# PlasmaControl/spectrogram-enhancement

Measured on AMD Instinct MI355X. Metric: spectrograms/s (STFT+VAE-denoise fwd) at 1/2/4/8 GPUs; PSNR vs CPU ref, higher is better.
Workload: dtype fp16; 1 GPU; BASELINE config 5 per GPU: end-to-end STFT -> SVD -> autoencoder-denoise inference stream, 16,512-sample fp16 shots -> specgr 128x128 (256 hann / hop 128) -> denoiseSignal default -> 3-layer conv AE (16/32/64, 5x5) fp16 forward -> fp16 reconstructions (32,768 B per shot); shots_per_launch=2048, samples=16512, stft_dtype=fp32, svd_dtype=fp32 (fp64 small algebra), ae_dtype=fp16, parallelism=shot-sharded x1, streams_per_gpu=2

## Files before the change

### spectrogram-enhancement_amd/csrc/decoder_tail.hip

```cpp
#include <hip/hip_runtime.h>

#include <algorithm>
#include <cstdlib>
#include <cstdint>
#include <string>
#include <type_traits>
#include <vector>

#include "lds_dma.hpp"
#include "specenh.h"
#include "runtime.hpp"
#include "wave.hpp"

namespace specenh {

namespace {

typedef _Float16 f16x8 __attribute__((ext_vector_type(8)));
typedef __bf16 bf16x8 __attribute__((ext_vector_type(8)));
typedef _Float16 f16x2 __attribute__((ext_vector_type(2)));
typedef __bf16 bf16x2 __attribute__((ext_vector_type(2)));
typedef float f32x4 __attribute__((ext_vector_type(4)));

constexpr int TO = 32;
// ... 500 lines not shown
  }
  if (i < ns) step(IC<0>{}, i, pa);
  if (i + 1 < ns) step(IC<1>{}, i + 1, pb);
  if (i + 2 < ns) step(IC<2>{}, i + 2, pa);
}

#ifndef SPECENH_D3_PEMIT
#define SPECENH_D3_PEMIT 0
#endif
namespace d3 {
constexpr int CI1 = 64, CO1 = 32;
constexpr int W1 = 32;
constexpr int X1ST = CI1;
constexpr int X1ROW = (W1 + 2) * X1ST;
constexpr int NX1 = 8;
constexpr int X2ST = 32;
constexpr int X2ROW = (2 * W1 + 2) * X2ST;
constexpr int NX2 = 8;
constexpr int LDS_X1 = NX1 * X1ROW * 2;
constexpr int LDS_X2 = NX2 * X2ROW * 2;
constexpr int LDS_M = rows::NMR * rows::MROW * 2;
constexpr int LDS_S = 4 * rows::SCR * rows::SCW * 4;
constexpr int LDS_BYTES = LDS_X1 + LDS_X2 + LDS_M + LDS_S;
constexpr int NBND = 6 * 2 * 4;
constexpr int BSTR = NBND + 64;
constexpr int LDS_ES = SPECENH_D3_PEMIT ? 2 * 2 * 4 * 64 * 4 : 0;
constexpr int LDS_BYTES_NM = LDS_X1 + LDS_X2 + 4 * BSTR * 4 + LDS_ES;
}

__device__ __forceinline__ int x1_off(int ps, int g) { return ps * d3::X1ST + 8 * (g ^ (ps & 7)); }

__device__ __forceinline__ int x2_off(int ps, int g) { return ps * d3::X2ST + 8 * (g ^ ((ps >> 1) & 3)); }


#ifndef SPECENH_D3_CPRIO
#define SPECENH_D3_CPRIO 1
#endif
#ifndef SPECENH_D3_BRANCHFREE
#define SPECENH_D3_BRANCHFREE 1
#endif

struct D3Args {
  const void* x;
  const void* w1;
  const float* b1;
  const void* wt;
  const float* bt;
  const void* wo;
  const float* bo;
  void* out;
  int N, H;
  int out_f16;
};

#ifdef SPECENH_D3_STATS
__device__ unsigned long long d3_stats[1024 * 8 * 4];
struct D3Clock {
  long long last = 0, busy = 0, wait = 0, n = 0;
  __device__ __forceinline__ void barrier() {
    asm volatile("s_waitcnt lgkmcnt(0)" ::: "memory");
    const long long t0 = __builtin_amdgcn_s_memtime();
    asm volatile("s_waitcnt lgkmcnt(0)" ::: "memory");
    __builtin_amdgcn_s_barrier();
    asm volatile("" ::: "memory");
    const long long t1 = __builtin_amdgcn_s_memtime();
    asm volatile("s_waitcnt lgkmcnt(0)" ::: "memory");
    if (last) busy += t0 - last;
    wait += t1 - t0;
    ++n;
    last = t1;
  }
  __device__ void flush(int wv) {
    if ((threadIdx.x & 63) == 0 && blockIdx.x < 1024) {
      unsigned long long* p = d3_stats + (blockIdx.x * 8 + wv) * 4;
      p[0] = busy; p[1] = wait; p[2] = n; p[3] = 0;
    }
  }
};
#define D3_BARRIER() clk.barrier()
#else
#define D3_BARRIER() lds_barrier()
#endif

template <typename T, bool MAP, int LEAD, bool OUT16 = false>
__global__ __launch_bounds__(512, 2) void decoder3_kernel(D3Args a) {
  static_assert(LEAD >= 0 && LEAD <= 4, "8-row input ring");
  using namespace d3;
  extern __shared__ __attribute__((aligned(16))) unsigned char lds_raw[];
  constexpr int LB = MAP ? LDS_BYTES : LDS_BYTES_NM;
  T* const x1r = reinterpret_cast<T*>(lds_raw);
  T* const x2r = reinterpret_cast<T*>(lds_raw + LDS_X1);
  T* const mr = reinterpret_cast<T*>(lds_raw + LDS_X1 + LDS_X2);
  float* const sc = reinterpret_cast<float*>(lds_raw + LDS_X1 + LDS_X2 + LDS_M);
  float* const bnd = reinterpret_cast<float*>(lds_raw + LDS_X1 + LDS_X2);
  float* const es = bnd + 4 * BSTR;

  const int tid = threadIdx.x, lane = tid & 63;
  const int wv = __builtin_amdgcn_readfirstlane(tid >> 6);
  const int m = lane & 15, kg = lane >> 4;
  const int H1 = a.H, H2 = 2 * H1, H3 = 4 * H1;
#ifdef SPECENH_D3_STATS
  D3Clock clk;
#endif
  const int SPI = H1 + 1, TPI = 2 * SPI;
  const int G = gridDim.x;
  const int nimg = ((int)a.N - (int)blockIdx.x + G - 1) / G;
  const int S = nimg * SPI + 2;
  {
    uint4* z = reinterpret_cast<uint4*>(lds_raw);
    for (int e = tid; e < LB / 16; e += 512) z[e] = uint4{0u, 0u, 0u, 0u};
  }
  __syncthreads();

  if (wv < 4) {
    const int wx = wv & 1, nb = wv >> 1;
    uint4 w1[50];
    {
      const T* __restrict__ Wg = reinterpret_cast<const T*>(a.w1);
      int u = 0;
#pragma unroll
      for (int ph = 0; ph < 4; ++ph)
#pragma unroll
        for (int dy = -1; dy <= 1; ++dy)
#pragma unroll
          for (int dx = -1; dx <= 1; ++dx) {
            const int ky = ky_of(ph >> 1, dy), kx = ky_of(ph & 1, dx);
            if (ky < 0 || ky >= KT || kx < 0 || kx >= KT) continue;
#pragma unroll
            for (int kh = 0; kh < 2; ++kh)
              w1[u++] = *reinterpret_cast<const uint4*>(
                  Wg + (((16 * nb + m) * KT + ky) * KT + kx) * CI1 + 32 * kh + 8 * kg);
          }
    }
    const f32x4 bias = f32x4{a.b1[16 * nb + 4 * kg], a.b1[16 * nb + 4 * kg + 1],
                             a.b1[16 * nb + 4 * kg + 2], a.b1[16 * nb + 4 * kg + 3]};
    resident_loads_landed();
    const T* __restrict__ X = reinterpret_cast<const T*>(a.x);
    const int dps = 1 + 8 * wv + (lane >> 3);
    const int dsrc = (dps - 1) * CI1 + 8 * ((lane & 7) ^ (dps & 7));
    unsigned char* const ddst = lds_raw + (1 + 8 * wv) * X1ST * 2;
    auto stage_at = [&](int p, int il, int row) -> bool {
      unsigned char* dst = ddst + (p & (NX1 - 1)) * X1ROW * 2;
      if (il < nimg && row >= 0 && row < H1) {
        const long long n = (long long)blockIdx.x + (long long)il * G;
        lds_dma16_s(X + ((n * H1 + row) * W1) * CI1, 2u * dsrc, dst);
        return true;
      }
      *reinterpret_cast<uint4*>(dst + 16 * lane) = uint4{0u, 0u, 0u, 0u};
      return false;
    };
    auto stage = [&](int p) -> bool {
      const int il = p / SPI;
      return stage_at(p, il, p - il * SPI - 1);
    };
    int xo[3];
#pragma unroll
    for (int dx = -1; dx <= 1; ++dx) xo[dx + 1] = x1_off(16 * wx + m + dx + 1, kg);
    const int x2w16 = x2_off(2 * (16 * wx + m) + 1 + (kg & 1), 2 * nb + (kg >> 1));
    auto store_pair = [&](T* row, uint2 p0, uint2 p1) {
      const auto sx = __builtin_amdgcn_permlane16_swap(p0.x, p1.x, false, false);
      const auto sy = __builtin_amdgcn_permlane16_swap(p0.y, p1.y, false, false);
      *reinterpret_cast<uint4*>(row + x2w16) = uint4{sx[0], sy[0], sx[1], sy[1]};
    };
#pragma unroll
    for (int p = 0; p < 3 + LEAD; ++p) stage(p);
    asm volatile("s_waitcnt vmcnt(0)" ::: "memory");
    D3_BARRIER();
    int vmn = 0;
// ... 73 lines not shown
      pstep(IC<6>{}, g + 6);
      pstep(IC<7>{}, g + 7);
    }
    if (g < S) pstep(IC<0>{}, g);
    if (g + 1 < S) pstep(IC<1>{}, g + 1);
    if (g + 2 < S) pstep(IC<2>{}, g + 2);
    if (g + 3 < S) pstep(IC<3>{}, g + 3);
    if (g + 4 < S) pstep(IC<4>{}, g + 4);
    if (g + 5 < S) pstep(IC<5>{}, g + 5);
    if (g + 6 < S) pstep(IC<6>{}, g + 6);
#ifdef SPECENH_D3_STATS
    clk.flush(wv);
#endif
  } else if constexpr (!MAP) {
    const int w = wv - 4;
    uint4 wt[25];
    {
      const T* __restrict__ Wt = reinterpret_cast<const T*>(a.wt);
      int u = 0;
#pragma unroll
      for (int ph = 0; ph < 4; ++ph)
#pragma unroll
        for (int dy = -1; dy <= 1; ++dy)
#pragma unroll
          for (int dx = -1; dx <= 1; ++dx) {
            const int ky = ky_of(ph >> 1, dy), kx = ky_of(ph & 1, dx);
            if (ky < 0 || ky >= KT || kx < 0 || kx >= KT) continue;
            wt[u++] = *reinterpret_cast<const uint4*>(Wt + ((m * KT + ky) * KT + kx) * CI + 8 * kg);
          }
    }
    const f32x4 bias = f32x4{a.bt[4 * kg], a.bt[4 * kg + 1], a.bt[4 * kg + 2], a.bt[4 * kg + 3]};
    uint4 wd[3][2];
    {
      const T* __restrict__ Wo = reinterpret_cast<const T*>(a.wo);
      const int i = lane & 15, kA = lane >> 4;
      const int gO = i >> 2, j = i & 3, r = gO >> 1, o = gO & 1;
      const int ox = o + (j == 1 ? 2 : (j == 2 ? -2 : 0));
#pragma unroll
      for (int d = 0; d < 3; ++d)
#pragma unroll
        for (int py = 0; py < 2; ++py) {
          const int ky = py + 2 - 2 * (d - 1) - r;
          uint32_t e[4];
#pragma unroll
          for (int h = 0; h < 4; ++h) {
            uint32_t v2 = 0;
#pragma unroll
            for (int s2 = 0; s2 < 2; ++s2) {
              const int el = 2 * h + s2, px = el >> 2, c = el & 3, kx = px + 2 - ox;
              unsigned short bits = 0;
              if (j < 3 && ky >= 0 && ky < KO && kx >= 0 && kx < KO)
                bits = __builtin_bit_cast(unsigned short, Wo[(ky * KO + kx) * CO + 4 * kA + c]);
              v2 |= (uint32_t)bits << (16 * s2);
            }
            e[h] = v2;
          }
          wd[d][py] = uint4{e[0], e[1], e[2], e[3]};
        }
    }
    const float bo = a.bo[0];
    resident_loads_landed();
    int xo[3];
#pragma unroll
    for (int dx = -1; dx <= 1; ++dx) xo[dx + 1] = x2_off(16 * w + m + dx + 1, kg);
    const int orow = kg >> 1, ocol = 32 * w + 2 * m + (kg & 1);
    const int bwi = (m == 0 || m == 15) ? ((w + 1) * 2 + (m == 0 ? 1 : 0)) * 4 + kg : NBND + lane;
    const int bri = m == 0 ? (w * 2 + 0) * 4 + kg : (m == 15 ? ((w + 2) * 2 + 1) * 4 + kg : 0);
#if SPECENH_D3_CPRIO
    __builtin_amdgcn_s_setprio(1);
#endif
    D3_BARRIER();

    f32x4 P0 = f32x4{0.f, 0.f, 0.f, 0.f}, P1 = P0, P2 = P0;
    int il = -1, tl = TPI - 4;
    auto frags = [&](auto ic, uint4 (&bq)[9]) {
      constexpr int T8 = decltype(ic)::value;
#pragma unroll
      for (int dy = -1; dy <= 1; ++dy)
#pragma unroll
        for (int dx = -1; dx <= 1; ++dx)
          bq[3 * (dy + 1) + dx + 1] =
              *reinterpret_cast<const uint4*>(x2r + ((T8 + dy + 8) & 7) * X2ROW + xo[dx + 1]);
    };
    auto tstep = [&](auto ic, const uint4 (&bq)[9], float* bb, f32x4& E, int& eil,
                     int& etl) -> bool {
      constexpr int T8 = decltype(ic)::value;
      (void)T8;
      eil = il;
      etl = tl;
      if (++tl == TPI) { tl = 0; ++il; }
      const bool img = eil >= 0 && eil < nimg;
#if !SPECENH_D3_BRANCHFREE
      if (!img) return false;
#endif
      f32x4 acc[4] = {bias, bias, bias, bias};
      int u0[4] = {0, 4, 10, 16};
#pragma unroll
      for (int dy = -1; dy <= 1; ++dy)
#pragma unroll
        for (int dx = -1; dx <= 1; ++dx) {
          const uint4 b = bq[3 * (dy + 1) + dx + 1];
#pragma unroll
          for (int ph = 0; ph < 4; ++ph) {
            const int ky = ky_of(ph >> 1, dy), kx = ky_of(ph & 1, dx);
            if (ky < 0 || ky >= KT || kx < 0 || kx >= KT) continue;
            acc[ph] = mfma<T>(wt[u0[ph]++], b, acc[ph]);
          }
        }
      const uint32_t keep = img && etl < H2 ? 0xffffffffu : 0u;
      uint4 bv[2];
#pragma unroll
      for (int py = 0; py < 2; ++py) {
        const uint2 lo = relu_pack<T>(acc[2 * py]), hi = relu_pack<T>(acc[2 * py + 1]);
        bv[py] = uint4{lo.x & keep, lo.y & keep, hi.x & keep, hi.y & keep};
      }
#pragma unroll
      for (int py = 0; py < 2; ++py) {
        P0 = mfma<T>(wd[0][py], bv[py], P0);
        P1 = mfma<T>(wd[1][py], bv[py], P1);
        P2 = mfma<T>(wd[2][py], bv[py], P2);
      }
      E = P0;
      P0 = P1;
      P1 = P2;
      P2 = f32x4{0.f, 0.f, 0.f, 0.f};
#if SPECENH_D3_BRANCHFREE
      bb[bwi] = m == 0 ? E[2] : E[1];
      return img && etl >= 1 && etl <= H2;
#else
      if (etl < 1 || etl > H2) return false;
      if (m == 0 || m == 15) bb[bwi] = m == 0 ? E[2] : E[1];
      return true;
#endif
    };
    auto tskip = [&](float* bb, f32x4& E, int& eil, int& etl) -> bool {
      eil = il;
      etl = tl;
      if (++tl == TPI) { tl = 0; ++il; }
      E = P0;
      P0 = P1;
      P1 = P2;
      P2 = f32x4{0.f, 0.f, 0.f, 0.f};
      bb[bwi] = m == 0 ? E[2] : E[1];
      return eil >= 0 && eil < nimg && etl >= 1 && etl <= H2;
    };
    auto emit = [&](const f32x4& E, float edge, int eil, int etl) {
      float s = bo + E[0];
      s += dpp_shift<0x111>(E[1]);
      s += dpp_shift<0x101>(E[2]);
      s += edge;
      const long long n = (long long)blockIdx.x + (long long)eil * G;
      const long long o = (n * H3 + 2 * (etl - 1) + orow) * rows::MW + ocol;
      const float y = __builtin_amdgcn_rcpf(1.f + __expf(-s));
      if constexpr (OUT16)
        reinterpret_cast<_Float16*>(a.out)[o] = (_Float16)y;
      else
        reinterpret_cast<float*>(a.out)[o] = y;
    };
    auto cstep = [&](auto ic) {
      constexpr int I = decltype(ic)::value;
      float* const b0 = bnd + ((I & 1) * 2) * BSTR;
      float* const b1 = b0 + BSTR;
      f32x4 E0, E1;
      int il0, tl0, il1, tl1;
      bool e0, e1;
      if (il >= 0 && il < nimg && tl < H2) {
        uint4 bq[9];
        frags(IC<(2 * I + 4) & 7>{}, bq);
        __builtin_amdgcn_sched_barrier(0);
        e0 = tstep(IC<(2 * I + 4) & 7>{}, bq, b0, E0, il0, tl0);
        frags(IC<(2 * I + 5) & 7>{}, bq);
        __builtin_amdgcn_sched_barrier(0);
        e1 = tstep(IC<(2 * I + 5) & 7>{}, bq, b1, E1, il1, tl1);
      } else {
        e0 = tskip(b0, E0, il0, tl0);
        e1 = tskip(b1, E1, il1, tl1);
      }
#if SPECENH_D3_PEMIT
      (void)e0;
      (void)e1;
      float* const ep = es + ((I & 1) * 2 * 4 + w) * 64 + lane;
      ep[0] = ((bo + E0[0]) + dpp_shift<0x111>(E0[1])) + dpp_shift<0x101>(E0[2]);
      ep[4 * 64] = ((bo + E1[0]) + dpp_shift<0x111>(E1[1])) + dpp_shift<0x101>(E1[2]);
      D3_BARRIER();
#else
      D3_BARRIER();
      if (e0) emit(E0, b0[bri], il0, tl0);
      if (e1) emit(E1, b1[bri], il1, tl1);
#endif
    };
    int g = 0;
    for (; g + 4 <= S; g += 4) {
      cstep(IC<0>{});
      cstep(IC<1>{});
      cstep(IC<2>{});
      cstep(IC<3>{});
    }
    if (g < S) cstep(IC<0>{});
    if (g + 1 < S) cstep(IC<1>{});
    if (g + 2 < S) cstep(IC<2>{});
#ifdef SPECENH_D3_STATS
    clk.flush(wv);
#endif
  } else {
    const int w = wv - 4;
    TailWave<T> tw;
    tw.load(a.wt, a.bt, a.wo, a.bo, w, lane);
    int xo[3];
#pragma unroll
    for (int dx = -1; dx <= 1; ++dx) xo[dx + 1] = x2_off(16 * w + m + dx + 1, kg);
    D3_BARRIER();
    auto tstep = [&](auto ic, const int t, float* scb) {
      constexpr int T8 = decltype(ic)::value;
      constexpr int T4 = T8 & 3;
      if (t < 0) return;
      const int il = t / TPI, tl = t - il * TPI;
      if (il >= nimg) return;
      if (tl >= 2)
        tw.conv_out_d([&](int j) { return mr + ((2 * T4 - 6 + j + 8) & 7) * rows::MROW; }, scb,
                      m);
      T* const m0 = mr + ((2 * T4) & 7) * rows::MROW;
      T* const m1 = mr + ((2 * T4 + 1) & 7) * rows::MROW;
      if (tl < H2)
        tw.convt(x2r, [](int dy) { return ((T8 + dy + 8) & 7) * X2ROW; },
                 [&](int dx) { return xo[dx + 1]; }, m0, m1);
      else
        tw.zero_rows(m0, m1);
    };
    auto sums = [&](const float* scb, int t) {
      if (t < 0) return;
      const int il = t / TPI, tl = t - il * TPI;
      if (il >= nimg || tl < 2) return;
      const long long n = (long long)blockIdx.x + (long long)il * G;
      tw.conv_out_sums(scb, reinterpret_cast<float*>(a.out) + n * H3 * rows::MW, 2 * tl - 4,
                       lane);
    };
    auto cstep = [&](auto ic, const int g) {
      constexpr int I = decltype(ic)::value;
      float* const sc0 = sc + ((I & 1) * 2) * (rows::SCR * rows::SCW);
      float* const sc1 = sc0 + rows::SCR * rows::SCW;
      tstep(IC<(2 * I + 5) & 7>{}, 2 * g - 3, sc0);
      tstep(IC<(2 * I + 6) & 7>{}, 2 * g - 2, sc1);
      D3_BARRIER();
      sums(sc0, 2 * g - 3);
      sums(sc1, 2 * g - 2);
    };
    int g = 0;
    for (; g + 4 <= S; g += 4) {
      cstep(IC<0>{}, g);
      cstep(IC<1>{}, g + 1);
      cstep(IC<2>{}, g + 2);
      cstep(IC<3>{}, g + 3);
    }
    if (g < S) cstep(IC<0>{}, g);
    if (g + 1 < S) cstep(IC<1>{}, g + 1);
    if (g + 2 < S) cstep(IC<2>{}, g + 2);
#ifdef SPECENH_D3_STATS
    clk.flush(wv);
#endif
  }
}

}
}

using namespace specenh;

namespace {
template <bool TRAIN>
int launch_tail_rows(int dtype, RowsArgs& r, hipStream_t st) {
  const int N = r.N, H = r.H;
  int nb = 1;
  while (nb < 8 && (long long)N * nb < 2ll * device_cus() && 2 * H / (2 * nb) >= 8) nb *= 2;
  r.R = ((2 * H + nb - 1) / nb + 1) & ~1;
  r.nb = (2 * H + r.R - 1) / r.R;
  const long long grid = (long long)N * r.nb;
  if (grid >= (1ll << 31)) return set_error(SPECENH_EINVAL, "too many workgroups");
  if (dtype == SPECENH_DTYPE_F16)
    SPECENH_LAUNCH((tail_rows_kernel<_Float16, TRAIN>), dim3((unsigned)grid), dim3(256), rows::LDS_BYTES, st, r);
  else
    SPECENH_LAUNCH((tail_rows_kernel<__bf16, TRAIN>), dim3((unsigned)grid), dim3(256), rows::LDS_BYTES, st, r);
  const hipError_t e = hipGetLastError();
  if (e != hipSuccess) return set_error(SPECENH_EHIP, std::string("tail_rows: ") + hipGetErrorString(e));
  return SPECENH_OK;
}
}

extern "C" int specenh_convt_conv_out_train(int dtype, const void* x, int N, int H, int W, int C,
                                            const void* wt_gemm, const float* bt, int CO_, int kt,
                                            const void* wo_gemm, const float* bo, int ko,
                                            void* map, float* logits, void* out, void* stream) {
  if (N < 0 || H <= 0 || W <= 0) return set_error(SPECENH_EINVAL, "bad input shape");
  if (dtype != SPECENH_DTYPE_F16 && dtype != SPECENH_DTYPE_BF16)
    return set_error(SPECENH_EUNSUPPORTED, "fused decoder tail: fp16 / bf16 only");
  if (C != CI || CO_ != CO || kt != KT || ko != KO || W != rows::QW)
    return set_error(SPECENH_EUNSUPPORTED,
                     "fused decoder tail (training): Conv2DTranspose(16, 5) on 64-wide "
                     "32-channel inputs + Conv2D(1, 5)");
  if (N == 0) return SPECENH_OK;
  if (!x || !wt_gemm || !bt || !wo_gemm || !bo || !map || !logits || !out)
    return set_error(SPECENH_EINVAL, "null pointer");
  if ((long long)N * H * W * C >= (1ll << 31) || (long long)N * 4 * H * W * CO >= (1ll << 31))
    return set_error(SPECENH_EINVAL, "tensor too large (2^31 elements)");
  RowsArgs r{};
  r.x = x; r.wt = wt_gemm; r.bt = bt; r.wo = wo_gemm; r.bo = bo;
  r.map = map; r.logits = logits; r.out_t = out;
  r.N = N; r.H = H;
  return launch_tail_rows<true>(dtype, r, (hipStream_t)stream);
}

namespace specenh {
bool tail_rows_general_supported(int C, int CO, int kt, int ko, int W);
int tail_rows_general(int dtype, const void* x, int N, int H, int W, int C, const void* wt,
                      const float* bt, int CO, int kt, const void* wo, const float* bo, int ko,
                      float* out, hipStream_t st, bool* launched);
}

extern "C" int specenh_convt_conv_out(int dtype, const void* x, int N, int H, int W, int C,
                                      const void* wt_gemm, const float* bt, int CO_, int kt,
                                      const void* wo_gemm, const float* bo, int ko, float* out,
                                      void* stream) {
  if (N < 0 || H <= 0 || W <= 0) return set_error(SPECENH_EINVAL, "bad input shape");
  if (dtype != SPECENH_DTYPE_F16 && dtype != SPECENH_DTYPE_BF16)
    return set_error(SPECENH_EUNSUPPORTED, "fused decoder tail: fp16 / bf16 only");
  hipStream_t st = (hipStream_t)stream;
  if (tail_rows_general_supported(C, CO_, kt, ko, W)) {
    if (N == 0) return SPECENH_OK;
    bool launched = false;
    const int rc = tail_rows_general(dtype, x, N, H, W, C, wt_gemm, bt, CO_, kt, wo_gemm, bo, ko,
                                     out, st, &launched);
    if (rc != SPECENH_OK || launched) return rc;
  }
  if (C != CI || CO_ != CO || kt != KT || ko != KO)
    return set_error(SPECENH_EUNSUPPORTED,
                     "fused decoder tail: Conv2DTranspose(16, 5) on 32 channels + Conv2D(1, 5), "
                     "or Conv2DTranspose(32, k) + Conv2D(1, k), k = 3 / 5 / 7, on 64-wide inputs");
  if (N == 0) return SPECENH_OK;
  if (W == rows::QW && variant(V_TAIL_TILES) == 0) {
    if (!x || !wt_gemm || !bt || !wo_gemm || !bo || !out) return set_error(SPECENH_EINVAL, "null pointer");
    if ((long long)N * H * W * C >= (1ll << 31) || (long long)N * 4 * H * W >= (1ll << 31))
      return set_error(SPECENH_EINVAL, "tensor too large (2^31 elements)");
    RowsArgs r{};
    r.x = x; r.wt = wt_gemm; r.bt = bt; r.wo = wo_gemm; r.bo = bo; r.out = out;
    r.N = N; r.H = H;
    return launch_tail_rows<false>(dtype, r, st);
  }
  if (!x || !wt_gemm || !bt || !wo_gemm || !bo || !out) return set_error(SPECENH_EINVAL, "null pointer");
  if ((long long)N * H * W * C >= (1ll << 31) || (long long)N * 4 * H * W >= (1ll << 31))
    return set_error(SPECENH_EINVAL, "tensor too large (2^31 elements)");
  TailArgs a{};
  a.x = x;
  a.wt = wt_gemm;
  a.bt = bt;
  a.wo = wo_gemm;
  a.bo = bo;
  a.out = out;
  a.N = N;
  a.H = H;
  a.W = W;
  a.tiles_y = (2 * H + TO - 1) / TO;
  a.tiles_x = (2 * W + TO - 1) / TO;
  const long long tiles = (long long)N * a.tiles_y * a.tiles_x;
  if (tiles >= (1ll << 31)) return set_error(SPECENH_EINVAL, "too many tiles");
  const unsigned grid = (unsigned)std::min<long long>(tiles, resident_grid());
  if (dtype == SPECENH_DTYPE_F16)
    SPECENH_LAUNCH(convt_conv_out_kernel<_Float16>, dim3(grid), dim3(512), 0, st, a);
  else
    SPECENH_LAUNCH(convt_conv_out_kernel<__bf16>, dim3(grid), dim3(512), 0, st, a);
  const hipError_t e = hipGetLastError();
  if (e != hipSuccess) return set_error(SPECENH_EHIP, std::string("convt_conv_out: ") +
                                                          hipGetErrorString(e));
  return SPECENH_OK;
}

#ifdef SPECENH_D3_STATS
extern "C" int specenh_d3_stats(void* host, int bytes) {
  return hipMemcpyFromSymbol(host, HIP_SYMBOL(d3_stats), bytes) == hipSuccess ? 0 : -1;
}
#endif

extern "C" int specenh_decoder3_ex(int dtype, const void* x, int N, int H, int W, int C,
                                   const void* w1_gemm, const float* b1, int CO1,
                                   const void* wt_gemm, const float* bt, int CO2,
                                   const void* wo_gemm, const float* bo, int k, void* out,
                                   int out_dtype, void* stream) {
  if (out_dtype != SPECENH_DTYPE_F32 && out_dtype != SPECENH_DTYPE_F16)
    return set_error(SPECENH_EUNSUPPORTED, "fused decoder: fp32 or fp16 output");
  if (N < 0 || H <= 0 || W <= 0) return set_error(SPECENH_EINVAL, "bad input shape");
  if (dtype != SPECENH_DTYPE_F16 && dtype != SPECENH_DTYPE_BF16)
    return set_error(SPECENH_EUNSUPPORTED, "fused decoder: fp16 / bf16 only");
  if (W != d3::W1 || C != d3::CI1 || CO1 != d3::CO1 || CO2 != CO || k != KT)
    return set_error(SPECENH_EUNSUPPORTED,
                     "fused decoder: Conv2DTranspose(32, 5) on 32-wide 64-channel inputs + "
                     "Conv2DTranspose(16, 5) + Conv2D(1, 5)");
  if (N == 0) return SPECENH_OK;
  if (!x || !w1_gemm || !b1 || !wt_gemm || !bt || !wo_gemm || !bo || !out)
    return set_error(SPECENH_EINVAL, "null pointer");
  if ((long long)N * H * W * C >= (1ll << 31) || (long long)N * 16 * H * W >= (1ll << 31))
    return set_error(SPECENH_EINVAL, "tensor too large (2^31 elements)");
  D3Args a{};
  a.x = x; a.w1 = w1_gemm; a.b1 = b1; a.wt = wt_gemm; a.bt = bt; a.wo = wo_gemm; a.bo = bo;
  a.out = out; a.N = N; a.H = H;
  a.out_f16 = out_dtype == SPECENH_DTYPE_F16;
  hipStream_t st = (hipStream_t)stream;
  static LdsOptIn lds_map, lds_nm;
  (void)allow_lds(lds_map,
                  {reinterpret_cast<const void*>(&decoder3_kernel<_Float16, true, 0>),
                   reinterpret_cast<const void*>(&decoder3_kernel<__bf16, true, 0>)},
                  d3::LDS_BYTES);
  (void)allow_lds(lds_nm,
                  {reinterpret_cast<const void*>(&decoder3_kernel<_Float16, false, 3>),
                   reinterpret_cast<const void*>(&decoder3_kernel<__bf16, false, 3>),
                   reinterpret_cast<const void*>(&decoder3_kernel<_Float16, false, 0>),
                   reinterpret_cast<const void*>(&decoder3_kernel<__bf16, false, 0>),
                   reinterpret_cast<const void*>(&decoder3_kernel<_Float16, false, 3, true>),
                   reinterpret_cast<const void*>(&decoder3_kernel<__bf16, false, 3, true>),
                   reinterpret_cast<const void*>(&decoder3_kernel<_Float16, false, 0, true>),
                   reinterpret_cast<const void*>(&decoder3_kernel<__bf16, false, 0, true>)},
                  d3::LDS_BYTES_NM);
  const unsigned grid = (unsigned)std::min<long long>(N, device_cus());
  const bool map = variant(V_D3_MAP) != 0, short_lead = variant(V_ROWS_SHORT_LEAD) != 0;
  if (map && a.out_f16)
    return set_error(SPECENH_EUNSUPPORTED, "fused decoder: the map consumer stores fp32 only");
  const dim3 gd(grid), bd(512);
  auto launch_nm = [&](auto t, auto o16) {
    using TT = decltype(t);
    constexpr bool O16 = decltype(o16)::value;
    if (short_lead)
      SPECENH_LAUNCH((decoder3_kernel<TT, false, 0, O16>), gd, bd, d3::LDS_BYTES_NM, st, a);
    else
      SPECENH_LAUNCH((decoder3_kernel<TT, false, 3, O16>), gd, bd, d3::LDS_BYTES_NM, st, a);
  };
  using F16OUT = std::integral_constant<bool, true>;
  using F32OUT = std::integral_constant<bool, false>;
  if (dtype == SPECENH_DTYPE_F16) {
    if (map)
      SPECENH_LAUNCH((decoder3_kernel<_Float16, true, 0>), gd, bd, d3::LDS_BYTES, st, a);
    else if (a.out_f16)
      launch_nm(_Float16{}, F16OUT{});
    else
      launch_nm(_Float16{}, F32OUT{});
  } else {
    if (map)
      SPECENH_LAUNCH((decoder3_kernel<__bf16, true, 0>), gd, bd, d3::LDS_BYTES, st, a);
    else if (a.out_f16)
      launch_nm(__bf16{}, F16OUT{});
    else
      launch_nm(__bf16{}, F32OUT{});
  }
  const hipError_t e = hipGetLastError();
  if (e != hipSuccess) return set_error(SPECENH_EHIP, std::string("decoder3: ") + hipGetErrorString(e));
  return SPECENH_OK;
}

extern "C" int specenh_decoder3(int dtype, const void* x, int N, int H, int W, int C,
                                const void* w1_gemm, const float* b1, int CO1, const void* wt_gemm,
                                const float* bt, int CO2, const void* wo_gemm, const float* bo,
                                int k, float* out, void* stream) {
  return specenh_decoder3_ex(dtype, x, N, H, W, C, w1_gemm, b1, CO1, wt_gemm, bt, CO2, wo_gemm, bo,
                             k, out, SPECENH_DTYPE_F32, stream);
}
```

### spectrogram-enhancement_amd/csrc/runtime.hip

```cpp
#include "runtime.hpp"

#include <algorithm>
#include <atomic>
#include <cstdlib>
#include <cstring>
#include <mutex>
#include <string>

#include "specenh.h"

namespace specenh {
namespace {

struct VariantName {
  const char* name;
  int dflt;
};
constexpr VariantName kVariants[V_COUNT] = {
    {"CONVT_PAIR", 0},      {"PATCH_NO_WL", 0},      {"PATCH_NO_K5", 0},
    {"PATCH_WSPLIT", -1},   {"CONV_NO_S2", 0},       {"CONV_NO_PATCH", 0},
    {"CONV_NO_C1MFMA", 0},  {"CONV_NO_NARROW", 0},   {"WGRAD_GENERIC", 0},
    {"WGRAD_NO_CO1", 0},    {"WGRAD_PERPHASE", 0},   {"SVD_GRAM_TILES", 0},
    {"TAIL_TILES", 0},      {"DECODER_UNFUSED", 0},  {"SVD_NO_TOP1", 0},
    {"CONV_NO_ROWS", 0},    {"CONVT_NO_ROWS", 0},    {"CONV1_NO_ROWS", 0},
    {"ENCODER_UNFUSED", 0},  {"STFT_NO_HOLD", 0},    {"D3_MAP", 0},
    {"ENC2_WPE2", 0},        {"CONVT_SHARED_RING", 0}, {"SVD_RECON_VALU", 0},
    {"ROWS_SHORT_LEAD", 0},  {"SVD_GRAM_F32", 0},
    {"SVD_RECON_BLOCKS", 0}, {"CONVT_PG", 0}, {"SVD_GZ_ROWS", 0}, {"EIG_SPLIT", 0}, {"CO1_VALU", 0},
    {"C1_MASK_MFMA", 1}, {"S2_MIN_NT", 2}, {"PATCH_MIN_WG", 512}, {"WGRAD_WG", 1024}, {"WGRAD_C1_TILES", 4},
    {"EIG_GRID", 32}, {"ROWS_BANDS", -1}, {"CONVT_STORE8", 0},
};

std::atomic<int> g_variant[V_COUNT];
std::once_flag g_variant_once;

void init_variants() {
  for (int i = 0; i < V_COUNT; ++i) {
    int v = kVariants[i].dflt;
    std::string env = std::string("SPECENH_") + kVariants[i].name;
    if (const char* s = std::getenv(env.c_str()); s && *s) v = std::atoi(s);
    g_variant[i].store(v, std::memory_order_relaxed);
  }
}

int variant_index(const char* name) {
  if (!name) return -1;
  if (std::strncmp(name, "SPECENH_", 8) == 0) name += 8;
  for (int i = 0; i < V_COUNT; ++i)
    if (std::strcmp(name, kVariants[i].name) == 0) return i;
  return -1;
}

constexpr int kMaxDevices = 64;
std::atomic<int> g_cus[kMaxDevices];

constexpr int kRing = 256;
thread_local const void* g_ring[kRing];
thread_local long long g_launches = 0;

thread_local std::string g_last_error;

}

int set_error(int code, const std::string& msg) {
  g_last_error = msg;
  return code;
}

int variant(Variant v) {
  std::call_once(g_variant_once, init_variants);
  return g_variant[v].load(std::memory_order_relaxed);
}

int device_cus() {
  int dev = 0;
  if (hipGetDevice(&dev) != hipSuccess || dev < 0 || dev >= kMaxDevices) return 256;
  int c = g_cus[dev].load(std::memory_order_relaxed);
  if (c > 0) return c;
  if (hipDeviceGetAttribute(&c, hipDeviceAttributeMultiprocessorCount, dev) != hipSuccess || c <= 0)
    c = 256;
  g_cus[dev].store(c, std::memory_order_relaxed);
  return c;
}

hipError_t allow_lds(LdsOptIn& site, std::initializer_list<const void*> kernels, int bytes) {
  static_assert(sizeof(site.done) / sizeof(site.done[0]) == kMaxDevices, "one flag per device");
  int dev = 0;
  hipError_t e = hipGetDevice(&dev);
  if (e != hipSuccess) return e;
  const bool known = dev >= 0 && dev < kMaxDevices;
  if (known && site.done[dev].load(std::memory_order_acquire)) return hipSuccess;
  for (const void* k : kernels) {
    hipFuncAttributes fa{};
    e = hipFuncGetAttributes(&fa, k);
    if (e != hipSuccess) return e;
    e = hipFuncSetAttribute(k, hipFuncAttributeMaxDynamicSharedMemorySize,
                            std::min(bytes, 160 * 1024 - (int)fa.sharedSizeBytes));
    if (e != hipSuccess) return e;
  }
  if (known) site.done[dev].store(true, std::memory_order_release);
  return hipSuccess;
}

void note_launch(const void* kernel) { g_ring[g_launches++ % kRing] = kernel; }

}

extern "C" {

const char* specenh_last_error(void) { return specenh::g_last_error.c_str(); }

int specenh_set_variant(const char* name, int value) {
  const int i = specenh::variant_index(name);
// ... 65 lines not shown
```

### spectrogram-enhancement_amd/csrc/runtime.hpp

```cpp
#pragma once

#include <hip/hip_runtime.h>

#include <atomic>
#include <initializer_list>
#include <string>

namespace specenh {

int set_error(int code, const std::string& msg);

inline int ilog2i(int n) {
  int l = 0;
  while ((1 << l) < n) ++l;
  return l;
}

enum Variant : int {
  V_CONVT_PAIR = 0,
  V_PATCH_NO_WL,
  V_PATCH_NO_K5,
  V_PATCH_WSPLIT,
  V_CONV_NO_S2,
  V_CONV_NO_PATCH,
  V_CONV_NO_C1MFMA,
  V_CONV_NO_NARROW,
  V_WGRAD_GENERIC,
  V_WGRAD_NO_CO1,
  V_WGRAD_PERPHASE,
  V_SVD_GRAM_TILES,
  V_TAIL_TILES,
  V_DECODER_UNFUSED,
  V_SVD_NO_TOP1,
  V_CONV_NO_ROWS,
  V_CONVT_NO_ROWS,
  V_CONV1_NO_ROWS,
  V_ENCODER_UNFUSED,
  V_STFT_NO_HOLD,
  V_D3_MAP,
  V_ENC2_WPE2,
  V_CONVT_SHARED_RING,
  V_SVD_RECON_VALU,
  V_ROWS_SHORT_LEAD,
  V_SVD_GRAM_F32,
  V_SVD_RECON_BLOCKS,
  V_CONVT_PG,
  V_SVD_GZ_ROWS,
  V_EIG_SPLIT,
  V_CO1_VALU,
  V_C1_MASK_MFMA,
  V_S2_MIN_NT,
  V_PATCH_MIN_WG,
  V_WGRAD_WG,
  V_WGRAD_C1_TILES,
  V_EIG_GRID,
  V_ROWS_BANDS,
  V_CONVT_STORE8,
  V_COUNT
};

int variant(Variant v);

int device_cus();

struct LdsOptIn {
  std::atomic<bool> done[64];
};
hipError_t allow_lds(LdsOptIn& site, std::initializer_list<const void*> kernels, int bytes);

void note_launch(const void* kernel);

}

#define SPECENH_LAUNCH(K, ...)                                        \
  do {                                                                \
    ::specenh::note_launch(reinterpret_cast<const void*>(&K));        \
    hipLaunchKernelGGL(K, __VA_ARGS__);                               \
  } while (0)
```

### spectrogram-enhancement_amd/csrc/svd_denoise.hip

```cpp
#include <hip/hip_runtime.h>

#include <algorithm>
#include <cmath>
#include <cstdlib>
#include <string>
#include <vector>

#include "fft_common.hpp"
#include "specenh.h"
#include "runtime.hpp"
#include "wave.hpp"

namespace specenh {

typedef float f32x16 __attribute__((ext_vector_type(16)));

struct XView {
  const float* base;
  long long batch_stride;
  long long sk, si;
};

__global__ __launch_bounds__(256) void gram_kernel(XView x, int K, int r, float* G,
                                                   int ntiles_side) {
// ... 2669 lines not shown
                          long long osi, long long nb, hipStream_t st) {
  static LdsOptIn lds_site;
  const hipError_t e = allow_lds(
      lds_site,
      {(const void*)recon_stream_kernel<KP, TO, true>, (const void*)recon_stream_kernel<KP, TO, false>,
       (const void*)recon_mfma_kernel<KP, TO>, (const void*)recon_kernel<KP, TO>},
      kMaxLds);
  if (e != hipSuccess) return e;
  if (variant(V_SVD_RECON_VALU) == 0) {
    constexpr int NT = (KP + 15) / 16, KPP = 16 * NT, KS = 2 * NT < 4 ? 2 : 1;
    const int RP = (r + 15) & ~15;
    const size_t lm = ((size_t)RP * (KPP + 1) + (size_t)RB * (RP + 2) +
                       (size_t)KS * RB * (KPP + 1)) * 4;
    const bool rowmaj16 = xb.si == 1 && r % 4 == 0 && xb.sk % 4 == 0 &&
                          xb.batch_stride % 4 == 0 && (reinterpret_cast<uintptr_t>(xb.base) & 15) == 0;
    const bool trans = xb.sk == 1 && xb.si != 1;
    if (lm <= kMaxLds && r <= 256 && (rowmaj16 || trans) &&
        variant(V_SVD_RECON_BLOCKS) == 0) {
      const int nblk = (Kr + RB - 1) / RB;
      const long long want = 4LL * device_cus();
      const int segs = (int)std::max(1LL, std::min<long long>(nblk, (want + nb - 1) / nb));
      const int bps = (nblk + segs - 1) / segs;
      const int grid_x = (nblk + bps - 1) / bps;
      if (trans)
        SPECENH_LAUNCH((recon_stream_kernel<KP, TO, true>), dim3(grid_x, (unsigned)nb), dim3(256),
                       lm, st, xb, Kr, r, V, K, lo, hi, comp, only, reinterpret_cast<TO*>(out),
                       ob, osk, osi, bps);
      else
        SPECENH_LAUNCH((recon_stream_kernel<KP, TO, false>), dim3(grid_x, (unsigned)nb), dim3(256),
                       lm, st, xb, Kr, r, V, K, lo, hi, comp, only, reinterpret_cast<TO*>(out),
                       ob, osk, osi, bps);
      return hipGetLastError();
    }
    if (lm <= kMaxLds) {
      SPECENH_LAUNCH((recon_mfma_kernel<KP, TO>), dim3((Kr + RB - 1) / RB, (unsigned)nb),
                     dim3(256), lm, st, xb, Kr, r, V, K, lo, hi, comp, only,
                     reinterpret_cast<TO*>(out), ob, osk, osi);
      return hipGetLastError();
    }
  }
  const size_t lds = (size_t)r * KP * 4 + (size_t)RB * (r + 1) * 4 + (size_t)RB * KP * 4;
  if (lds > kMaxLds) return hipErrorInvalidValue;
  SPECENH_LAUNCH((recon_kernel<KP, TO>), dim3((Kr + RB - 1) / RB, (unsigned)nb), dim3(256),
                     lds, st, xb, Kr, r, V, K, lo, hi, comp, only, reinterpret_cast<TO*>(out),
                     ob, osk, osi);
  return hipGetLastError();
}

template <typename TO>
hipError_t launch_recon_k(int KP, XView xb, int Kr, int r, const float* V, int K, int lo,
                          int hi, int comp, const int* only, void* out, long long ob,
                          long long osk, long long osi, long long nb, hipStream_t st) {
  switch (KP) {
#define SPECENH_RC(n)                                                                          \
  case n:                                                                                      \
    return launch_recon_t<n, TO>(xb, Kr, r, V, K, lo, hi, comp, only, out, ob, osk, osi, nb, \
                                 st);
    SPECENH_RC(8) SPECENH_RC(16) SPECENH_RC(24) SPECENH_RC(32) SPECENH_RC(40) SPECENH_RC(48)
#undef SPECENH_RC
    default: return hipErrorInvalidValue;
  }
}

size_t dtype_size(int dt) { return dt == SPECENH_DTYPE_F32 ? 4 : 2; }

struct EigLayout {
  int r;
  long long ld;
  size_t per_matrix() const {
    return (size_t)r * r * 8 + 3 * (size_t)r * 8 + 4 * (size_t)r * ld * 8 + 4 * 4 + 8;
  }
  static constexpr size_t kCapBytes = 1ull << 30;
  long long chunk(long long batch) const {
    const long long c = (long long)(kCapBytes / per_matrix());
    return std::max(1LL, std::min(batch, c));
  }
  size_t bytes(long long batch) const { return (size_t)chunk(batch) * per_matrix() + 256; }
};
EigLayout eig_layout(int r) { return EigLayout{r, (long long)(r / 2 + 2)}; }

#ifndef SPECENH_EIG_MERGED
#define SPECENH_EIG_MERGED 1
#endif
template <typename TO>
__global__ __launch_bounds__(256) void eig_fallback_kernel(
    XView x, int Kr, int r, double* G, int nts, double* dg, double* eg, double* taug, int lo,
    int hi, double* Z, double* fac, long long ld, int* kinfo, TO* out, long long out_bstride,
    long long osk, long long osi, const int* only, long long nmat) {
  const int ntri = nts * (nts + 1) / 2, nkb = (Kr + RB - 1) / RB;
  for (long long b = blockIdx.x; b < nmat; b += gridDim.x) {
    if (!only[b]) continue;
    for (int t = 0; t < ntri; ++t) {
      gram64_one(x, Kr, r, G, nts, b, t);
      __syncthreads();
    }
    __threadfence();
    __syncthreads();
    tridiag_one(G, r, dg, eg, taug, b);
    __threadfence();
    __syncthreads();
    eigvec_one(G, dg, eg, taug, r, lo, hi, nullptr, Z, fac, ld, kinfo, b);
    __threadfence();
    __syncthreads();
    for (int kb = 0; kb < nkb; ++kb) {
      recon_eig_one<TO>(x, Kr, r, Z, ld, kinfo, out, out_bstride, osk, osi, b, kb);
      __syncthreads();
    }
  }
}

constexpr size_t recon_eig_lds(int r) {
  return (size_t)RB * (r + 1) * 4 + (size_t)r * 33 * 4 + (size_t)RB * 33 * 4;
}

template <typename TO>
hipError_t launch_recon_eig_t(XView xb, int Kr, int r, const double* Z, long long ld,
                              const int* kinfo, void* out, long long ob, long long osk,
                              long long osi, long long nb, hipStream_t st, const int* only) {
  const size_t lds = recon_eig_lds(r);
  static LdsOptIn lds_site;
  hipError_t e =
      allow_lds(lds_site, {(const void*)recon_eig_kernel<TO>}, (int)recon_eig_lds(EIG_MAXN));
  if (e != hipSuccess) return e;
  const unsigned gm = only ? (unsigned)std::min<long long>(nb, 2LL * device_cus()) : (unsigned)nb;
  SPECENH_LAUNCH(recon_eig_kernel<TO>, dim3((Kr + RB - 1) / RB, gm), dim3(256), lds, st, xb, Kr,
                 r, Z, ld, kinfo, reinterpret_cast<TO*>(out), ob, osk, osi, only, nb);
  return hipGetLastError();
}

template <typename TO>
hipError_t launch_eig_fallback_t(XView xb, int Kr, int r, double* G, int nts, double* dg,
                                 double* eg, double* taug, int lo, int hi, double* Z,
                                 double* fac, long long ld, int* kinfo, void* out, long long ob,
                                 long long osk, long long osi, const int* only, long long nb,
                                 unsigned gm, hipStream_t st) {
  const size_t lds = recon_eig_lds(r);
  static LdsOptIn lds_site;
  hipError_t e =
      allow_lds(lds_site, {(const void*)eig_fallback_kernel<TO>}, (int)recon_eig_lds(EIG_MAXN));
  if (e != hipSuccess) return e;
  SPECENH_LAUNCH(eig_fallback_kernel<TO>, dim3(gm), dim3(256), lds, st, xb, Kr, r, G, nts, dg,
                 eg, taug, lo, hi, Z, fac, ld, kinfo, reinterpret_cast<TO*>(out), ob, osk, osi,
                 only, nb);
  return hipGetLastError();
}

struct Oriented {
  XView xv;
  int Kr;
  long long osk, osi;
};
Oriented orient(const float* A, int m, int n, long long a_stride) {
  if (m >= n) return {{A, a_stride, n, 1}, m, n, 1};
  return {{A, a_stride, 1, n}, n, 1, n};
}

int eig_denoise(const float* A, long long batch, int m, int n, long long a_stride, int lo,
                int hi, int opt_mode, void* out, int odt, int* num_out, double* med_out,
                int* bad, void* workspace, hipStream_t st, const int* only = nullptr) {
  const int r = std::min(m, n);
  if (r > EIG_MAXN)
    return set_error(SPECENH_EUNSUPPORTED,
                     "kept range needs the eigen path, which handles min(m, n) <= 256");
  const EigLayout L = eig_layout(r);
  const long long ch = L.chunk(batch);
  char* w = (char*)workspace;
  double* G64 = (double*)w;
  double* dd = G64 + ch * (long long)r * r;
  double* ee = dd + ch * r;
  double* tau = ee + ch * r;
  double* Z = tau + ch * r;
  double* fac = Z + ch * (long long)r * L.ld;
  int* kinfo = (int*)(fac + 3 * ch * (long long)r * L.ld);
  int* ranges = kinfo + 2 * ch;
  int* num = ranges + 2 * ch;
  double* med = (double*)(((uintptr_t)(num + ch) + 7) & ~(uintptr_t)7);
  const Oriented o = orient(A, m, n, a_stride);
  XView xv = o.xv;
  const int Kr = o.Kr;
  const long long osk = o.osk, osi = o.osi;
  const long long ob = (long long)m * n;
  const size_t osz = dtype_size(odt);
  const int nts64 = (r + 63) / 64, ntri64 = nts64 * (nts64 + 1) / 2;
  const double beta = (double)r / (double)std::max(m, n);
  const double omega = ((0.0 + 0.56 * std::pow(beta, 3.0)) + -0.95 * std::pow(beta, 2.0)) +
                       1.82 * std::pow(beta, 1.0) + 1.43 * std::pow(beta, 0.0);
  for (long long b0 = 0; b0 < batch; b0 += ch) {
    const long long nb = std::min(ch, batch - b0);
    xv.base = A + b0 * a_stride;
    const int* on = only ? only + b0 : nullptr;
    void* ob0 = static_cast<char*>(out) + (size_t)(b0 * ob) * osz;
    const long long gcap = variant(V_EIG_GRID) > 0 ? variant(V_EIG_GRID) : 2LL * device_cus();
    const unsigned gm = on ? (unsigned)std::min<long long>(nb, gcap) : (unsigned)nb;
    const bool merged_fits = (long long)r * Kr <= 128LL * 128;
    if (on && opt_mode < 0 && merged_fits && SPECENH_EIG_MERGED && variant(V_EIG_SPLIT) == 0) {
      const hipError_t e = with_out_type(odt, [&](auto t) {
        return launch_eig_fallback_t<decltype(t)>(xv, Kr, r, G64, nts64, dd, ee, tau, lo, hi, Z,
                                                  fac, L.ld, kinfo, ob0, ob, osk, osi, on, nb, gm,
                                                  st);
      });
      if (e != hipSuccess) return set_error(SPECENH_EHIP, std::string("eigen fallback: ") + hipGetErrorString(e));
      continue;
    }
    SPECENH_LAUNCH(gram64_kernel, dim3(ntri64, gm), dim3(256), 0, st, xv, Kr, r, G64, nts64, on,
                   nb);
    SPECENH_LAUNCH(tridiag_kernel, dim3(gm), dim3(256), 0, st, G64, r, dd, ee, tau, on, nb);
    const int* rg = nullptr;
    if (opt_mode >= 0) {
      SPECENH_LAUNCH(optimal_rank_kernel, dim3((unsigned)nb), dim3(64), 0, st, dd, ee, r,
                         omega, num, med);
      SPECENH_LAUNCH(optimal_ranges_kernel, dim3((unsigned)((nb + 255) / 256)), dim3(256), 0,
                         st, num, nb, r, opt_mode, ranges, bad);
      if (num_out && hipMemcpyAsync(num_out + b0, num, (size_t)nb * 4, hipMemcpyDeviceToDevice,
                                    st) != hipSuccess)
        return set_error(SPECENH_EHIP, "num_sing copy");
      if (med_out && hipMemcpyAsync(med_out + b0, med, (size_t)nb * 8, hipMemcpyDeviceToDevice,
                                    st) != hipSuccess)
        return set_error(SPECENH_EHIP, "median copy");
      rg = ranges;
    }
    SPECENH_LAUNCH(eigvec_kernel, dim3(gm), dim3(256), 0, st, G64, dd, ee, tau, r, lo, hi, rg,
                   Z, fac, L.ld, kinfo, on, nb);
    if (hipGetLastError() != hipSuccess) return set_error(SPECENH_EHIP, "eigen path launch");
    const hipError_t e = with_out_type(odt, [&](auto t) {
      return launch_recon_eig_t<decltype(t)>(xv, Kr, r, Z, L.ld, kinfo, ob0, ob, osk, osi, nb, st,
                                             on);
// ... 253 lines not shown
```

Before: 1.975 million spectrograms/s.

## Software-pipeline decoder3 conv loop and ballot-scan eig fallback matrix list

The decoder3 conv-transpose waves now prefetch the next row's B fragments and the previous step's edge values in the middle of the current step's MFMA chain. The sigmoid emit of the previous step is deferred into the gap after the second MFMA group, with output offsets tracked incrementally. This hides LDS latency and the exp/rcp/store work behind matrix math, at the cost of more live registers and more complex index bookkeeping. The eig fallback kernel also uses a wave ballot to compact the list of flagged matrices 256 at a time, so it no longer loads the per-matrix flag serially before each matrix. The old paths stay available behind new variant flags.

Result: no change. 1.995 million spectrograms/s, median of 6 (+1.0%).

```diff
diff --git a/spectrogram-enhancement_amd/csrc/decoder_tail.hip b/spectrogram-enhancement_amd/csrc/decoder_tail.hip
--- a/spectrogram-enhancement_amd/csrc/decoder_tail.hip
+++ b/spectrogram-enhancement_amd/csrc/decoder_tail.hip
@@ -606,8 +606,8 @@
 #define D3_BARRIER() lds_barrier()
 #endif
 
-template <typename T, bool MAP, int LEAD, bool OUT16 = false>
-__global__ __launch_bounds__(512, 2) void decoder3_kernel(D3Args a) {
+template <typename T, bool MAP, int LEAD, bool OUT16, bool SERIAL>
+__device__ __forceinline__ void decoder3_body(const D3Args& a) {
   static_assert(LEAD >= 0 && LEAD <= 4, "8-row input ring");
   using namespace d3;
   extern __shared__ __attribute__((aligned(16))) unsigned char lds_raw[];
@@ -847,8 +847,8 @@
           bq[3 * (dy + 1) + dx + 1] =
               *reinterpret_cast<const uint4*>(x2r + ((T8 + dy + 8) & 7) * X2ROW + xo[dx + 1]);
     };
-    auto tstep = [&](auto ic, const uint4 (&bq)[9], float* bb, f32x4& E, int& eil,
-                     int& etl) -> bool {
+    auto tstep = [&](auto ic, uint4 (&bq)[9], float* bb, f32x4& E, int& eil, int& etl, auto&& mid,
+                     auto&& hole) -> bool {
       constexpr int T8 = decltype(ic)::value;
       (void)T8;
       eil = il;
@@ -872,12 +872,12 @@
             acc[ph] = mfma<T>(wt[u0[ph]++], b, acc[ph]);
           }
         }
-      const uint32_t keep = img && etl < H2 ? 0xffffffffu : 0u;
+      mid();
       uint4 bv[2];
 #pragma unroll
       for (int py = 0; py < 2; ++py) {
         const uint2 lo = relu_pack<T>(acc[2 * py]), hi = relu_pack<T>(acc[2 * py + 1]);
-        bv[py] = uint4{lo.x & keep, lo.y & keep, hi.x & keep, hi.y & keep};
+        bv[py] = uint4{lo.x, lo.y, hi.x, hi.y};
       }
 #pragma unroll
       for (int py = 0; py < 2; ++py) {
@@ -885,6 +885,7 @@
         P1 = mfma<T>(wd[1][py], bv[py], P1);
         P2 = mfma<T>(wd[2][py], bv[py], P2);
       }
+      hole();
       E = P0;
       P0 = P1;
       P1 = P2;
@@ -922,6 +923,7 @@
       else
         reinterpret_cast<float*>(a.out)[o] = y;
     };
+    auto nothing = [] {};
     auto cstep = [&](auto ic) {
       constexpr int I = decltype(ic)::value;
       float* const b0 = bnd + ((I & 1) * 2) * BSTR;
@@ -933,10 +935,10 @@
         uint4 bq[9];
         frags(IC<(2 * I + 4) & 7>{}, bq);
         __builtin_amdgcn_sched_barrier(0);
-        e0 = tstep(IC<(2 * I + 4) & 7>{}, bq, b0, E0, il0, tl0);
+        e0 = tstep(IC<(2 * I + 4) & 7>{}, bq, b0, E0, il0, tl0, nothing, nothing);
         frags(IC<(2 * I + 5) & 7>{}, bq);
         __builtin_amdgcn_sched_barrier(0);
-        e1 = tstep(IC<(2 * I + 5) & 7>{}, bq, b1, E1, il1, tl1);
+        e1 = tstep(IC<(2 * I + 5) & 7>{}, bq, b1, E1, il1, tl1, nothing, nothing);
       } else {
         e0 = tskip(b0, E0, il0, tl0);
         e1 = tskip(b1, E1, il1, tl1);
@@ -954,16 +956,97 @@
       if (e1) emit(E1, b1[bri], il1, tl1);
 #endif
     };
+    using OT = std::conditional_t<OUT16, _Float16, float>;
+    const uint32_t lane_off = (uint32_t)(orow * rows::MW + ocol);
+    const long long wrapd = ((long long)G * H3 - 2 * (TPI - 2)) * rows::MW;
+    long long ob = (((long long)blockIdx.x - G) * H3 + 2 * (TPI - 5)) * rows::MW;
+    uint4 bq[9];
+    float ps0 = 0.f, ps1 = 0.f;
+    bool pe0 = false, pe1 = false;
+    long long pob = 0;
+    auto part = [&](const f32x4& E) {
+      float s = bo + E[0];
+      s += dpp_shift<0x111>(E[1]);
+      s += dpp_shift<0x101>(E[2]);
+      return s;
+    };
+    auto emit_p = [&](float s, float edge, long long o) {
+      s += edge;
+      const float y = __builtin_amdgcn_rcpf(1.f + __expf(-s));
+      (reinterpret_cast<OT*>(a.out) + o)[lane_off] = (OT)y;
+    };
+    auto cstep_p = [&](auto ic) {
+      constexpr int I = decltype(ic)::value;
+      float* const b0 = bnd + ((I & 1) * 2) * BSTR;
+      float* const b1 = b0 + BSTR;
+      const float* const q0 = bnd + (((I + 1) & 1) * 2) * BSTR;
+      float g0, g1;
+      auto edges = [&] { g0 = q0[bri]; g1 = q0[BSTR + bri]; };
+      auto flush0 = [&] { if (pe0) emit_p(ps0, g0, pob); };
+      auto flush1 = [&] { if (pe1) emit_p(ps1, g1, pob + 2 * rows::MW); };
+      f32x4 E0, E1;
+      int il0, tl0, il1, tl1;
+      bool e0, e1;
+      float n0, n1;
+      const long long onow = ob;
+      if (il >= 0 && il < nimg && tl < H2) {
+        e0 = tstep(IC<(2 * I + 4) & 7>{}, bq, b0, E0, il0, tl0,
+                   [&] {
+                     __builtin_amdgcn_sched_barrier(0);
+                     edges();
+                     frags(IC<(2 * I + 5) & 7>{}, bq);
+                     __builtin_amdgcn_sched_barrier(0);
+                   },
+                   flush0);
+        n0 = part(E0);
+        e1 = tstep(IC<(2 * I + 5) & 7>{}, bq, b1, E1, il1, tl1,
+                   [&] {
+                     __builtin_amdgcn_sched_barrier(0);
+                     frags(IC<(2 * I + 6) & 7>{}, bq);
+                     __builtin_amdgcn_sched_barrier(0);
+                   },
+                   flush1);
+        n1 = part(E1);
+      } else {
+        edges();
+        frags(IC<(2 * I + 6) & 7>{}, bq);
+        flush0();
+        flush1();
+        e0 = tskip(b0, E0, il0, tl0);
+        n0 = part(E0);
+        e1 = tskip(b1, E1, il1, tl1);
+        n1 = part(E1);
+      }
+      ps0 = n0; ps1 = n1; pe0 = e0; pe1 = e1; pob = onow;
+      ob += tl == 0 ? wrapd : 4 * rows::MW;
+      D3_BARRIER();
+    };
     int g = 0;
-    for (; g + 4 <= S; g += 4) {
-      cstep(IC<0>{});
-      cstep(IC<1>{});
-      cstep(IC<2>{});
-      cstep(IC<3>{});
+    if constexpr (SERIAL || SPECENH_D3_PEMIT) {
+      for (; g + 4 <= S; g += 4) {
+        cstep(IC<0>{});
+        cstep(IC<1>{});
+        cstep(IC<2>{});
+        cstep(IC<3>{});
+      }
+      if (g < S) cstep(IC<0>{});
+      if (g + 1 < S) cstep(IC<1>{});
+      if (g + 2 < S) cstep(IC<2>{});
+    } else {
+      frags(IC<4>{}, bq);
+      for (; g + 4 <= S; g += 4) {
+        cstep_p(IC<0>{});
+        cstep_p(IC<1>{});
+        cstep_p(IC<2>{});
+        cstep_p(IC<3>{});
+      }
+      if (g < S) cstep_p(IC<0>{});
+      if (g + 1 < S) cstep_p(IC<1>{});
+      if (g + 2 < S) cstep_p(IC<2>{});
+      const float* const q0 = bnd + (((S - 1) & 1) * 2) * BSTR;
+      if (pe0) emit_p(ps0, q0[bri], pob);
+      if (pe1) emit_p(ps1, q0[BSTR + bri], pob + 2 * rows::MW);
     }
-    if (g < S) cstep(IC<0>{});
-    if (g + 1 < S) cstep(IC<1>{});
-    if (g + 2 < S) cstep(IC<2>{});
 #ifdef SPECENH_D3_STATS
     clk.flush(wv);
 #endif
@@ -1024,6 +1107,16 @@
     clk.flush(wv);
 #endif
   }
+}
+
+template <typename T, bool MAP, int LEAD, bool OUT16 = false>
+__global__ __launch_bounds__(512, 2) void decoder3_kernel(D3Args a) {
+  decoder3_body<T, MAP, LEAD, OUT16, false>(a);
+}
+
+template <typename T, int LEAD, bool OUT16>
+__global__ __launch_bounds__(512, 2) void decoder3_serial_kernel(D3Args a) {
+  decoder3_body<T, false, LEAD, OUT16, true>(a);
 }
 
 }
@@ -1181,17 +1274,30 @@
                    reinterpret_cast<const void*>(&decoder3_kernel<_Float16, false, 3, true>),
                    reinterpret_cast<const void*>(&decoder3_kernel<__bf16, false, 3, true>),
                    reinterpret_cast<const void*>(&decoder3_kernel<_Float16, false, 0, true>),
-                   reinterpret_cast<const void*>(&decoder3_kernel<__bf16, false, 0, true>)},
+                   reinterpret_cast<const void*>(&decoder3_kernel<__bf16, false, 0, true>),
+                   reinterpret_cast<const void*>(&decoder3_serial_kernel<_Float16, 3, false>),
+                   reinterpret_cast<const void*>(&decoder3_serial_kernel<__bf16, 3, false>),
+                   reinterpret_cast<const void*>(&decoder3_serial_kernel<_Float16, 0, false>),
+                   reinterpret_cast<const void*>(&decoder3_serial_kernel<__bf16, 0, false>),
+                   reinterpret_cast<const void*>(&decoder3_serial_kernel<_Float16, 3, true>),
+                   reinterpret_cast<const void*>(&decoder3_serial_kernel<__bf16, 3, true>),
+                   reinterpret_cast<const void*>(&decoder3_serial_kernel<_Float16, 0, true>),
+                   reinterpret_cast<const void*>(&decoder3_serial_kernel<__bf16, 0, true>)},
                   d3::LDS_BYTES_NM);
   const unsigned grid = (unsigned)std::min<long long>(N, device_cus());
   const bool map = variant(V_D3_MAP) != 0, short_lead = variant(V_ROWS_SHORT_LEAD) != 0;
+  const bool serial = variant(V_D3_SERIAL) != 0;
   if (map && a.out_f16)
     return set_error(SPECENH_EUNSUPPORTED, "fused decoder: the map consumer stores fp32 only");
   const dim3 gd(grid), bd(512);
   auto launch_nm = [&](auto t, auto o16) {
     using TT = decltype(t);
     constexpr bool O16 = decltype(o16)::value;
-    if (short_lead)
+    if (serial && short_lead)
+      SPECENH_LAUNCH((decoder3_serial_kernel<TT, 0, O16>), gd, bd, d3::LDS_BYTES_NM, st, a);
+    else if (serial)
+      SPECENH_LAUNCH((decoder3_serial_kernel<TT, 3, O16>), gd, bd, d3::LDS_BYTES_NM, st, a);
+    else if (short_lead)
       SPECENH_LAUNCH((decoder3_kernel<TT, false, 0, O16>), gd, bd, d3::LDS_BYTES_NM, st, a);
     else
       SPECENH_LAUNCH((decoder3_kernel<TT, false, 3, O16>), gd, bd, d3::LDS_BYTES_NM, st, a);
diff --git a/spectrogram-enhancement_amd/csrc/runtime.hip b/spectrogram-enhancement_amd/csrc/runtime.hip
--- a/spectrogram-enhancement_amd/csrc/runtime.hip
+++ b/spectrogram-enhancement_amd/csrc/runtime.hip
@@ -28,7 +28,7 @@
     {"ROWS_SHORT_LEAD", 0},  {"SVD_GRAM_F32", 0},
     {"SVD_RECON_BLOCKS", 0}, {"CONVT_PG", 0}, {"SVD_GZ_ROWS", 0}, {"EIG_SPLIT", 0}, {"CO1_VALU", 0},
     {"C1_MASK_MFMA", 1}, {"S2_MIN_NT", 2}, {"PATCH_MIN_WG", 512}, {"WGRAD_WG", 1024}, {"WGRAD_C1_TILES", 4},
-    {"EIG_GRID", 32}, {"ROWS_BANDS", -1}, {"CONVT_STORE8", 0},
+    {"EIG_GRID", 32}, {"ROWS_BANDS", -1}, {"CONVT_STORE8", 0}, {"D3_SERIAL", 0}, {"EIG_SERIAL_SCAN", 0},
 };
 
 std::atomic<int> g_variant[V_COUNT];
diff --git a/spectrogram-enhancement_amd/csrc/runtime.hpp b/spectrogram-enhancement_amd/csrc/runtime.hpp
--- a/spectrogram-enhancement_amd/csrc/runtime.hpp
+++ b/spectrogram-enhancement_amd/csrc/runtime.hpp
@@ -56,6 +56,8 @@
   V_EIG_GRID,
   V_ROWS_BANDS,
   V_CONVT_STORE8,
+  V_D3_SERIAL,
+  V_EIG_SERIAL_SCAN,
   V_COUNT
 };
 
diff --git a/spectrogram-enhancement_amd/csrc/svd_denoise.hip b/spectrogram-enhancement_amd/csrc/svd_denoise.hip
--- a/spectrogram-enhancement_amd/csrc/svd_denoise.hip
+++ b/spectrogram-enhancement_amd/csrc/svd_denoise.hip
@@ -2775,30 +2775,78 @@
 #ifndef SPECENH_EIG_MERGED
 #define SPECENH_EIG_MERGED 1
 #endif
+struct EigFallbackArgs {
+  XView x;
+  int Kr, r;
+  double* G;
+  int nts;
+  double *dg, *eg, *taug;
+  int lo, hi;
+  double *Z, *fac;
+  long long ld;
+  int* kinfo;
+  long long out_bstride, osk, osi;
+};
+
+template <typename TO>
+__device__ __forceinline__ void eig_fallback_one(const EigFallbackArgs& a, TO* out, long long b) {
+  const int ntri = a.nts * (a.nts + 1) / 2, nkb = (a.Kr + RB - 1) / RB;
+  for (int t = 0; t < ntri; ++t) {
+    gram64_one(a.x, a.Kr, a.r, a.G, a.nts, b, t);
+    __syncthreads();
+  }
+  __threadfence();
+  __syncthreads();
+  tridiag_one(a.G, a.r, a.dg, a.eg, a.taug, b);
+  __threadfence();
+  __syncthreads();
+  eigvec_one(a.G, a.dg, a.eg, a.taug, a.r, a.lo, a.hi, nullptr, a.Z, a.fac, a.ld, a.kinfo, b);
+  __threadfence();
+  __syncthreads();
+  for (int kb = 0; kb < nkb; ++kb) {
+    recon_eig_one<TO>(a.x, a.Kr, a.r, a.Z, a.ld, a.kinfo, out, a.out_bstride, a.osk, a.osi, b, kb);
+    __syncthreads();
+  }
+}
+
 template <typename TO>
 __global__ __launch_bounds__(256) void eig_fallback_kernel(
     XView x, int Kr, int r, double* G, int nts, double* dg, double* eg, double* taug, int lo,
     int hi, double* Z, double* fac, long long ld, int* kinfo, TO* out, long long out_bstride,
     long long osk, long long osi, const int* only, long long nmat) {
-  const int ntri = nts * (nts + 1) / 2, nkb = (Kr + RB - 1) / RB;
+  const EigFallbackArgs a{x, Kr, r, G, nts, dg, eg, taug, lo, hi, Z, fac, ld, kinfo, out_bstride, osk, osi};
+  __shared__ int s_list[256];
+  __shared__ int s_cnt[4];
+  const int tid = threadIdx.x, wave = tid >> 6, lane = tid & 63;
+  for (long long i0 = 0; (long long)blockIdx.x + i0 * gridDim.x < nmat; i0 += 256) {
+    const long long b = (long long)blockIdx.x + (i0 + tid) * gridDim.x;
+    const bool on = b < nmat && only[b] != 0;
+    const unsigned long long mask = __ballot(on);
+    if (lane == 0) s_cnt[wave] = __popcll(mask);
+    __syncthreads();
+    int base = 0, total = 0;
+#pragma unroll
+    for (int v = 0; v < 4; ++v) {
+      const int c = s_cnt[v];
+      base += v < wave ? c : 0;
+      total += c;
+    }
+    if (on) s_list[base + __popcll(mask & ((1ull << lane) - 1ull))] = tid;
+    __syncthreads();
+    for (int k = 0; k < total; ++k)
+      eig_fallback_one<TO>(a, out, (long long)blockIdx.x + (i0 + s_list[k]) * gridDim.x);
+  }
+}
+
+template <typename TO>
+__global__ __launch_bounds__(256) void eig_fallback_serial_kernel(
+    XView x, int Kr, int r, double* G, int nts, double* dg, double* eg, double* taug, int lo,
+    int hi, double* Z, double* fac, long long ld, int* kinfo, TO* out, long long out_bstride,
+    long long osk, long long osi, const int* only, long long nmat) {
+  const EigFallbackArgs a{x, Kr, r, G, nts, dg, eg, taug, lo, hi, Z, fac, ld, kinfo, out_bstride, osk, osi};
   for (long long b = blockIdx.x; b < nmat; b += gridDim.x) {
     if (!only[b]) continue;
-    for (int t = 0; t < ntri; ++t) {
-      gram64_one(x, Kr, r, G, nts, b, t);
-      __syncthreads();
-    }
-    __threadfence();
-    __syncthreads();
-    tridiag_one(G, r, dg, eg, taug, b);
-    __threadfence();
-    __syncthreads();
-    eigvec_one(G, dg, eg, taug, r, lo, hi, nullptr, Z, fac, ld, kinfo, b);
-    __threadfence();
-    __syncthreads();
-    for (int kb = 0; kb < nkb; ++kb) {
-      recon_eig_one<TO>(x, Kr, r, Z, ld, kinfo, out, out_bstride, osk, osi, b, kb);
-      __syncthreads();
-    }
+    eig_fallback_one<TO>(a, out, b);
   }
 }
 
@@ -2829,12 +2877,18 @@
                                  unsigned gm, hipStream_t st) {
   const size_t lds = recon_eig_lds(r);
   static LdsOptIn lds_site;
-  hipError_t e =
-      allow_lds(lds_site, {(const void*)eig_fallback_kernel<TO>}, (int)recon_eig_lds(EIG_MAXN));
+  hipError_t e = allow_lds(
+      lds_site, {(const void*)eig_fallback_kernel<TO>, (const void*)eig_fallback_serial_kernel<TO>},
+      (int)recon_eig_lds(EIG_MAXN));
   if (e != hipSuccess) return e;
-  SPECENH_LAUNCH(eig_fallback_kernel<TO>, dim3(gm), dim3(256), lds, st, xb, Kr, r, G, nts, dg,
-                 eg, taug, lo, hi, Z, fac, ld, kinfo, reinterpret_cast<TO*>(out), ob, osk, osi,
-                 only, nb);
+  if (variant(V_EIG_SERIAL_SCAN) != 0)
+    SPECENH_LAUNCH(eig_fallback_serial_kernel<TO>, dim3(gm), dim3(256), lds, st, xb, Kr, r, G, nts,
+                   dg, eg, taug, lo, hi, Z, fac, ld, kinfo, reinterpret_cast<TO*>(out), ob, osk,
+                   osi, only, nb);
+  else
+    SPECENH_LAUNCH(eig_fallback_kernel<TO>, dim3(gm), dim3(256), lds, st, xb, Kr, r, G, nts, dg,
+                   eg, taug, lo, hi, Z, fac, ld, kinfo, reinterpret_cast<TO*>(out), ob, osk, osi,
+                   only, nb);
   return hipGetLastError();
 }
 
```
